# Sawyerbatch/simglucose

Measured on AMD Instinct MI355X. Metric: env-steps/sec at batch=1M patients (1-min dt); fp64 glucose trace max-abs-err, higher is better.
Workload: dtype f64

## Files before the change

### simglucose_amd/csrc/t1d_kernels.hpp

```cpp
#pragma once
#include "../../include/t1d.h"
#include "t1d_device.hpp"

#ifndef T1D_WAVES
#define T1D_WAVES 2
#endif
#ifndef T1D_ROW_RECOMPUTE
#define T1D_ROW_RECOMPUTE 1
#endif
constexpr int kFlagReverse = 0x10000;
#ifndef T1D_AB_FLAGS
#define T1D_AB_FLAGS 0
#endif

#include <climits>
#include <cstdint>
#include <type_traits>

namespace t1d {

template <typename T> struct KArgs {
    int64_t n, env_offset;
    uint64_t seed;
    T* x; T* planned; T* last_qsto; T* last_food; int32_t* t; uint32_t* meta; uint32_t* episode; int32_t* next_meal;
// ... 91 lines not shown
template <typename T>
__device__ __forceinline__ void stage_prop(const KArgs<T>& a, T* lds)
{
    const int tot = a.prop_rows * a.np_pad;
    for (int j = threadIdx.x; j < tot; j += blockDim.x) lds[j] = a.prop[j];
    __syncthreads();
}

template <typename T>
__device__ __forceinline__ void load_env(const KArgs<T>& a, unsigned i, uint32_t meta, Env<T>& e)
{
#pragma unroll
    for (int k = 0; k < 13; ++k) e.x[k] = at(row(a.x, a.n, k), i);
    e.planned = at(a.planned, i); e.lq = at(a.last_qsto, i); e.lf = at(a.last_food, i);
    e.last_cgm = at(a.last_cgm, i); e.prev_risk = at(a.prev_risk, i);
#pragma unroll
    for (int k = 0; k < 4; ++k) e.cur[k] = at(row(a.pts, a.n, 22 + k), i);
    e.t = at(a.t, i);
    e.next_meal = a.next_meal ? at(a.next_meal, i) : 0;
    e.next_meal_loaded = e.next_meal;
    e.eating = (meta & T1D_META_EATING) != 0;
    e.cursor = (int)T1D_META_CURSOR(meta);
}

template <typename T>
__device__ __forceinline__ void store_env(const KArgs<T>& a, unsigned i, uint32_t pid, const Env<T>& e)
{
#pragma unroll
    for (int k = 0; k < 13; ++k) at(row(a.x, a.n, k), i) = e.x[k];
    at(a.planned, i) = e.planned; at(a.last_qsto, i) = e.lq; at(a.last_food, i) = e.lf;
    at(a.last_cgm, i) = e.last_cgm; at(a.prev_risk, i) = e.prev_risk;
    if (a.dbar) at(a.dbar, i) = dbar_of(e.lq, e.lf);
    at(a.t, i) = e.t;
    if (a.next_meal && e.next_meal != e.next_meal_loaded) at(a.next_meal, i) = e.next_meal;
    at(a.meta, i) = pid | (e.eating ? T1D_META_EATING : 0u) | (e.planned > T(0) ? T1D_META_PLANNED : 0u) | ((uint32_t)e.cursor << 16);
}

constexpr int kPtsRows = 26;
constexpr int kPackedRows = 18 + kPtsRows + 1;
constexpr int kRowDbar = 18 + kPtsRows;

#ifndef T1D_REFILL_INLINE
#define T1D_REFILL_INLINE 1
#endif
#if T1D_REFILL_INLINE
#define T1D_REFILL_ATTR __forceinline__
#else
#define T1D_REFILL_ATTR __noinline__
#endif

template <typename T>
__device__ T1D_REFILL_ATTR void noise_refill(T* __restrict__ pts, const T* __restrict__ normals, const T* __restrict__ minv,
                                             const uint32_t* __restrict__ episode, int* status, int64_t n, unsigned i,
                                             int64_t env_offset, uint64_t seed, int n_normals, int b, SensorC<T> sen, T* ar_e)
{
    const T p0 = at(rowv(pts, n, b > 0 ? 10 : 0), i);
    at(pts, i) = p0;
    T M[11];
#pragma unroll
    for (int k = 0; k < 11; ++k) M[k] = minv[k * 11] * p0;
    T e = *ar_e;
    const uint32_t ep = (!normals && episode) ? at(episode, i) : 0u;
#pragma unroll 1
    for (int q = 0; q < 5; ++q) {
        T z0, z1;
        if (normals) {
            const int d = 1 + 10 * b + 2 * q;
            if (d + 1 < n_normals) { z0 = at(rowv(normals, n, d), i); z1 = at(rowv(normals, n, d + 1), i); }
            else { z0 = z1 = T(0); atomicOr(status, T1D_ST_NORMALS_EXHAUSTED); }
        } else {
            const double2 r = philox_pair(seed, (uint64_t)(env_offset + i), ep, 3u + 5u * (uint32_t)b + (uint32_t)q);
            z0 = (T)r.x; z1 = (T)r.y;
        }
        e = sen.pacf * (e + z0);
        const T ya = johnson_su<true>(sen, e);
        e = sen.pacf * (e + z1);
        const T yb = johnson_su<true>(sen, e);
        at(rowv(pts, n, 2 * q + 1), i) = ya;
        at(rowv(pts, n, 2 * q + 2), i) = yb;
        const T* mc = minv + (2 * q + 1);
#pragma unroll
        for (int k = 0; k < 11; ++k) M[k] += mc[k * 11] * ya + mc[k * 11 + 1] * yb;
    }
    *ar_e = e;
#pragma unroll
    for (int k = 0; k < 11; ++k) at(rowv(pts, n, 11 + k), i) = M[k];
}

__device__ __forceinline__ void divmod_uniform(int x, int d, int& q, int& r)
{
    switch (d) {
        case 1: q = x; r = 0; return;
        case 3: q = x / 3; break;
        case 5: q = x / 5; break;
        case 30: q = x / 30; break;
        case 50: q = x / 50; break;
        case 150: q = x / 150; break;
        default: q = x / d; break;
    }
    r = x - q * d;
}

template <bool REFILL, typename T>
__device__ __forceinline__ T noise_sample(const KArgs<T>& a, unsigned i, int s, T (&cur)[4], bool* entered = nullptr)
{
    const int64_t n = a.n;
    const int st = a.sen.st;
    int j, b;
    divmod_uniform(s, a.S, b, j);
    const int tau = (j + 1) * st;
    const int m = tau / 15 < 9 ? tau / 15 : 9;
    const int mprev = (tau - st) / 15 < 9 ? (tau - st) / 15 : 9;
    if (REFILL && j == 0) {
        T e = at(a.ar_e, i);
        noise_refill<T>(a.pts, a.normals, a.minv, a.episode, a.status, n, i, a.env_offset, a.seed, a.n_normals, b, a.sen, &e);
        at(a.ar_e, i) = e;
    }
    if (j == 0 || m != mprev) {
        cur[0] = at(rowv(a.pts, n, m), i);      cur[1] = at(rowv(a.pts, n, m + 1), i);
        cur[2] = at(rowv(a.pts, n, 11 + m), i); cur[3] = at(rowv(a.pts, n, 12 + m), i);
        if (entered) *entered = true;
        else {
#pragma unroll
            for (int k = 0; k < 4; ++k) at(row(a.pts, n, 22 + k), i) = cur[k];
        }
    }
    const T B = T(tau - 15 * m) * T(1.0 / 15.0), A = fma(-T(tau - 15 * m), T(1.0 / 15.0), T(1));
    const T ca = fma(A * A, A, -A), cb = fma(B * B, B, -B);
    return fma(A, cur[0], fma(B, cur[1], T(37.5) * fma(ca, cur[2], cb * cur[3])));
}

template <bool REFILL, typename T>
__device__ __forceinline__ T measure_noise(const KArgs<T>& a, unsigned i, Env<T>& e, bool& due, bool* entered = nullptr)
{
    const int t1 = e.t + 1;
    int q, r;
    divmod_uniform(t1, a.sen.st, q, r);
    due = r == 0;
    return due ? noise_sample<REFILL>(a, i, 1 + q, e.cur, entered) : T(0);
}
template <typename T>
__device__ __forceinline__ T measure_apply(const KArgs<T>& a, Env<T>& e, T gsub, T noise, bool due)
{
    if (due) {
        T cgm = gsub + noise;
        cgm = cgm > a.sen.vmin ? cgm : a.sen.vmin;
        cgm = cgm < a.sen.vmax ? cgm : a.sen.vmax;
        e.last_cgm = cgm;
    }
    return e.last_cgm;
}

template <typename T, bool HAS_NEXT = false, typename E = Env<T>>
__device__ __forceinline__ T meal_lookup(const KArgs<T>& a, unsigned i, E& e)
{
    T meal = T(0);
    if (HAS_NEXT || a.next_meal) {
        if (e.next_meal <= e.t) {
            while (e.cursor < a.n_meals) {
                const int mt = at(rowv(a.meal_time, a.n, e.cursor), i);
                if (mt > e.t) { e.next_meal = mt; break; }
                if (mt == e.t) meal = at(rowv(a.meal_amt, a.n, e.cursor), i);
                ++e.cursor;
            }
            if (e.cursor >= a.n_meals) e.next_meal = INT_MAX;
            asm volatile("" : "+v"(meal));
        }
    } else if (e.cursor < a.n_meals) {
        int mt = at(rowv(a.meal_time, a.n, e.cursor), i);
        while (mt < e.t && ++e.cursor < a.n_meals) mt = at(rowv(a.meal_time, a.n, e.cursor), i);
        if (e.cursor < a.n_meals && mt == e.t) {
            meal = at(rowv(a.meal_amt, a.n, e.cursor), i);
            ++e.cursor;
        }
    }
    return meal;
}

template <int MATH, typename T, typename P, bool REFILL = true, typename PR = NoProp, bool TIERED = false>
__device__ __forceinline__ StepOut<T> step_body(const KArgs<T>& a, P& p, unsigned i, Env<T>& e,
                                                T basal, T bolus, bool has_bolus, PR pr = PR())
{
    T q_basal, q_bolus;
    if ((a.flags & T1D_BATCH_NO_PUMP) || ab_flag(a, 0x200)) {
        q_basal = basal; q_bolus = has_bolus ? bolus : T(0);
    } else {
        q_basal = pump_quantise(basal, a.pump.inc_basal, a.pump.min_basal, a.pump.max_basal);
        q_bolus = a.pump.min_bolus > T(0) ? a.pump.min_bolus : T(0);
        if (has_bolus) q_bolus = pump_quantise(bolus, a.pump.inc_bolus, a.pump.min_bolus, a.pump.max_bolus);
    }
    const T insulin = q_basal + q_bolus;
    const T div = T(a.minutes), inv_div = T(1) / div;
    StepOut<T> o{T(0), T(0), T(0), T(0)};
    for (int m = 0; m < a.minutes; ++m) {
        const T meal = a.cho ? at(row(a.cho, a.n, m), i) : meal_lookup(a, i, e);
        bool due;
        const T noise = ab_flag(a, 0x400) ? (due = false, T(0)) : measure_noise<REFILL>(a, i, e, due);
        MinuteIn<T> u = eat_minute<MATH, T>(p, e.x, meal, insulin, e.planned, e.lq, e.lf, e.eating);
        if constexpr (PR::kSplit) p.pin_split(); else p.pin();
        if (!ab_flag(a, 0x800)) {
            if constexpr (PR::kSplit && TIERED) split_minute_tiered(p, pr, u, e.x, a.n_sub);
            else if constexpr (PR::kSplit) split_level<1>(p, pr, u, e.x, a.n_sub);
            else rk4_minute<MATH>(p, u, e.x, a.n_sub);
        }
        e.t += 1;
        const T gsub = MATH == 0 ? e.x[12] / p(DP_VG) : e.x[12] * p(DP_IVG);
        const T cgm = measure_apply(a, e, gsub, noise, due);
        if (MATH == 0) { o.meal += meal / div; o.ins += insulin / div; o.bg += gsub / div; o.cgm += cgm / div; }
        else { o.meal += meal * inv_div; o.ins += insulin * inv_div; o.bg += gsub * inv_div; o.cgm += cgm * inv_div; }
    }
    if (MATH != 0 && a.minutes == 1) { o.ins = insulin; }
    return o;
}

template <int MATH, typename T>
__device__ __forceinline__ void write_outputs(const KArgs<T>& a, unsigned i, Env<T>& e, const StepOut<T>& o, T rp)
{
    T l, h, r, rc = T(0);
    if (!ab_flag(a, 0x100)) risk_index1<MATH>(o.cgm, l, h, rc);
    at(a.reward, i) = rp - rc;
    e.prev_risk = rc;
    at(a.cgm, i) = o.cgm; at(a.bg, i) = o.bg;
    at(a.done, i) = (o.bg < T(70) || o.bg > T(350)) ? 1 : 0;
    if (a.lbgi || a.hbgi || a.risk) {
        risk_index1<MATH>(o.bg, l, h, r);
        if (a.lbgi) at(a.lbgi, i) = l;
        if (a.hbgi) at(a.hbgi, i) = h;
        if (a.risk) at(a.risk, i) = r;
    }
    if (a.meal) at(a.meal, i) = o.meal;
    if (a.insulin) at(a.insulin, i) = o.ins;
    if (!(fabs((double)e.x[12]) <= 1.0e300)) atomicOr(a.status, T1D_ST_NONFINITE);
}

template <int VARIANT> struct VariantMath { static constexpr int value = VARIANT == 0 ? 0 : 1; };
template <int VARIANT> struct VariantInfo {
    static_assert(VARIANT == 0 || VARIANT == 3 || VARIANT == 4 || VARIANT == 6 || VARIANT == 7, "unknown kernel variant");
    static constexpr bool split = VARIANT == 4 || VARIANT == 6 || VARIANT == 7;
    static constexpr bool tiered = VARIANT == 6 || VARIANT == 7;
    static constexpr bool lds_pars = VARIANT == 0 || VARIANT == 7;
};
extern __shared__ __align__(16) unsigned char t1d_dyn_lds[];

template <int VARIANT, typename T, bool REFILL = true>
__global__ __launch_bounds__(kBlock, T1D_WAVES) void step_kernel(const KArgs<T> a)
{
    constexpr int MATH = VariantMath<VARIANT>::value;
    using VI = VariantInfo<VARIANT>;
    constexpr int kParRows = VI::split ? DP_COUNT : DP_RK4_COUNT;
    __shared__ T lds[VI::lds_pars ? kParRows * kMaxPatients : 1];
    if (VI::lds_pars) stage_pars(a, lds, kParRows);
    if (VI::split) stage_prop(a, (T*)t1d_dyn_lds);
    const unsigned i = blockIdx.x * kBlock + threadIdx.x;
    __builtin_assume(i < (1u << 28));
    if ((int64_t)i >= a.n) return;
    const uint32_t meta = at(a.meta, i);
    const uint32_t pid = T1D_META_PID(meta);
    Env<T> e;
    load_env(a, i, meta, e);
    const T basal = at(a.basal, i);
    const T bolus = a.bolus ? at(a.bolus, i) : T(0);
    const T rp = e.prev_risk;
    StepOut<T> o;
    if constexpr (VARIANT == 4 || VARIANT == 6) {
        ParsReg<T> p;
        p.load(a.dpar, (int)pid);
        o = step_body<MATH, T, ParsReg<T>, REFILL, PropLds<T>, VARIANT == 6>(a, p, i, e, basal, bolus, a.bolus != nullptr, PropLds<T>{(const T*)t1d_dyn_lds, a.np_pad, (int)pid});
    } else if constexpr (VARIANT == 7) {
        ParsLds<T> p{lds, (int)pid};
        o = step_body<MATH, T, ParsLds<T>, REFILL, PropLds<T>, true>(a, p, i, e, basal, bolus, a.bolus != nullptr, PropLds<T>{(const T*)t1d_dyn_lds, a.np_pad, (int)pid});
    } else if constexpr (VARIANT == 3) {
        ParsReg<T> p;
        p.load(a.dpar, (int)pid);
        o = step_body<MATH, T, ParsReg<T>, REFILL>(a, p, i, e, basal, bolus, a.bolus != nullptr);
    } else {
        ParsLds<T> p{lds, (int)pid};
        o = step_body<MATH, T, ParsLds<T>, REFILL>(a, p, i, e, basal, bolus, a.bolus != nullptr);
    }
    write_outputs<MATH>(a, i, e, o, rp);
    store_env(a, i, pid, e);
}

#ifndef T1D_S1_WAVES
#define T1D_S1_WAVES 3
#endif
#ifndef T1D_S1_TRACE
#define T1D_S1_TRACE 0
#endif
#ifndef T1D_S1_PHASE_PRIO
#define T1D_S1_PHASE_PRIO 3
#endif
#if T1D_S1_TRACE
#define S1_MARK(m) do { __builtin_amdgcn_s_waitcnt(0x0070); if (tr && (threadIdx.x & 63) == 0 && tk < 6) tr[tk * 8 + (m)] = (long long)wall_clock64(); } while (0)
#else
#define S1_MARK(m) do { } while (0)
#endif
template <typename T> constexpr int s1_threads();
#ifndef T1D_S1D_WAVES
#define T1D_S1D_WAVES 4
#endif
#ifndef T1D_S1D_WAVES_F32
#define T1D_S1D_WAVES_F32 4
#endif
template <typename T> constexpr int s1d_threads() { return 256 * (sizeof(T) == 4 ? T1D_S1D_WAVES_F32 : T1D_S1D_WAVES); }
template <typename T> constexpr int s1_threads() { return 256 * (sizeof(T) == 4 ? T1D_S1D_WAVES_F32 : T1D_S1_WAVES); }
template <typename T> struct S1In { uint32_t meta; int t, next_meal; T basal, bolus, planned, lq, lf, x[13]; };

template <typename T>
__device__ __forceinline__ S1In<T> s1_load(const KArgs<T>& a, unsigned i)
{
    const BRows<T> X(a.x, a.n, kPackedRows);
    const BRows<int32_t> I(a.t, a.n, 3);
    S1In<T> in;
    in.meta = (uint32_t)(int32_t)at(I(1), i);
    in.t = at(I(0), i);
    in.next_meal = at(I(2), i);
    in.basal = at(a.basal, i);
    in.bolus = a.bolus ? (T)at(a.bolus, i) : T(0);
    const T dbar = at(X(kRowDbar), i);
#pragma unroll
    for (int k = 0; k < 13; ++k) in.x[k] = at(X(k), i);
    if ((in.meta & (T1D_META_EATING | T1D_META_PLANNED)) || (T1D_AB_FLAGS && (a.flags & 0x1000))) {
        in.planned = at(X(13), i); in.lq = at(X(14), i); in.lf = at(X(15), i);
    } else {
        in.planned = T(0); in.lq = dbar; in.lf = T(0);
    }
    return in;
}

constexpr int kS1DPark = 128;
template <typename T>
__device__ __forceinline__ void s1_park(const S1In<T>& in, T* pt, int* pi, int slot)
{
#pragma unroll
    for (int k = 0; k < 13; ++k) pt[k * kS1DPark + slot] = in.x[k];
    pt[13 * kS1DPark + slot] = in.planned; pt[14 * kS1DPark + slot] = in.lq; pt[15 * kS1DPark + slot] = in.lf;
    pt[16 * kS1DPark + slot] = in.basal; pt[17 * kS1DPark + slot] = in.bolus;
    pi[slot] = (int)in.meta; pi[kS1DPark + slot] = in.t; pi[2 * kS1DPark + slot] = in.next_meal;
}
template <typename T>
__device__ __forceinline__ S1In<T> s1_unpark(const T* pt, const int* pi, int slot)
{
    S1In<T> in;
#pragma unroll
    for (int k = 0; k < 13; ++k) in.x[k] = pt[k * kS1DPark + slot];
    in.planned = pt[13 * kS1DPark + slot]; in.lq = pt[14 * kS1DPark + slot]; in.lf = pt[15 * kS1DPark + slot];
    in.basal = pt[16 * kS1DPark + slot]; in.bolus = pt[17 * kS1DPark + slot];
    in.meta = (uint32_t)pi[slot]; in.t = pi[kS1DPark + slot]; in.next_meal = pi[2 * kS1DPark + slot];
    return in;
}

template <typename T, int MODE> constexpr bool kS1DLean = sizeof(T) == 8 && (MODE == 2 || MODE == 3);
constexpr int kLcVmin = 6, kLcVmax = 7, kLcLimits = 8, kLcHc1 = kLcLimits, kLcHc2 = kLcHc1 + 5, kLcSize = kLcHc2 + 5;
constexpr int kLcHc(int level) { return level == 1 ? kLcHc1 : kLcHc2; }
template <typename T>
__device__ __forceinline__ void pump_lconst(const T* lconst, T basal, T bolus, bool has_bolus, T& q_basal, T& q_bolus)
{
    int z = 0;
    asm volatile("" : "+v"(z));
    const T* lc = lconst + z;
    q_basal = pump_quantise(basal, lc[0], lc[1], lc[2]);
    q_bolus = lc[4] > T(0) ? lc[4] : T(0);
    if (has_bolus) q_bolus = pump_quantise(bolus, lc[3], lc[4], lc[5]);
}
template <bool REG, typename T, int STRIDE, bool EXTRA, int MODE, typename ONLEVEL>
__device__ __forceinline__ void s1_chunk(const KArgs<T>& a, T* ldp, T* lpr, T* lconst, unsigned i, const S1In<T>& in,
                                         ONLEVEL&& on_level, long long* tr, int tk)
{
    constexpr int LEVEL = MODE == 3 ? 2 : 1;
    (void)tr; (void)tk;
    S1_MARK(0);
    const BRows<T> X(a.x, a.n, kPackedRows);
    const BRows<int32_t> I(a.t, a.n, 3);
    const uint32_t meta = in.meta;
    Env<T> e;
    e.t = in.t;
    e.next_meal = in.next_meal;
    const T basal = in.basal;
    const T bolus = in.bolus;
    e.planned = in.planned; e.lq = in.lq; e.lf = in.lf;
#pragma unroll
    for (int k = 0; k < 13; ++k) e.x[k] = in.x[k];
    const uint32_t pid = T1D_META_PID(meta);
    const T planned0 = e.planned, lq0 = e.lq, lf0 = e.lf;
    e.next_meal_loaded = e.next_meal;
    e.eating = (meta & T1D_META_EATING) != 0;
    e.cursor = (int)T1D_META_CURSOR(meta);
    S1_MARK(1);
    T q_basal, q_bolus;
    if (a.flags & T1D_BATCH_NO_PUMP) {
        q_basal = basal; q_bolus = a.bolus ? bolus : T(0);
    } else {
        pump_lconst(lconst, basal, bolus, a.bolus != nullptr, q_basal, q_bolus);
    }
    const T insulin = q_basal + q_bolus;
    T meal;
    if (a.cho) {
        meal = at(a.cho, i);
        asm volatile("" : "+v"(meal));
    } else {
        meal = meal_lookup<T, true>(a, i, e);
    }
    ParsLdsS<T, STRIDE> pl{ldp, (int)pid};
    MinuteIn<T> u = eat_minute<1, T>(pl, e.x, meal, insulin, e.planned, e.lq, e.lf, e.eating);
    T f1 = T(0);
    if (MODE == 2) {
        const TierPre<T> tp = tier_pre(pl, u, e.x);
        f1 = tp.f1;
        on_level(tp.level2);
        if (tp.level2) return;
    }
    {
        const bool live0 = (meta & (T1D_META_EATING | T1D_META_PLANNED)) != 0 || (T1D_AB_FLAGS && (a.flags & 0x1000));
        const bool changed = live0 ? (e.planned != planned0 || e.lq != lq0 || e.lf != lf0) : (e.eating || e.planned > T(0));
        if (changed) {
            at(X(13), i) = e.planned; at(X(14), i) = e.lq; at(X(15), i) = e.lf;
            at(X(kRowDbar), i) = dbar_of(e.lq, e.lf);
        }
    }
    at(I(0), i) = e.t + 1;
    if (e.next_meal != e.next_meal_loaded) at(I(2), i) = e.next_meal;
    {
        const uint32_t meta1 = pid | (e.eating ? T1D_META_EATING : 0u) | (e.planned > T(0) ? T1D_META_PLANNED : 0u) | ((uint32_t)e.cursor << 16);
        if (meta1 != meta) at(I(1), i) = (int32_t)meta1;
    }
    if (EXTRA) {
        if (a.meal) at(a.meal, i) = meal;
        if (a.insulin) at(a.insulin, i) = insulin;
    }
    S1_MARK(2);
#if T1D_S1_PHASE_PRIO
    if (MODE != 3) __builtin_amdgcn_s_setprio(0);
#endif
    if (!ab_flag(a, 0x800)) {
        PropLdsS<T, STRIDE> pr{lpr, (int)pid};
        if (MODE == 1) {
            split_minute_tiered(pl, pr, u, e.x, a.n_sub);
        } else if constexpr (kS1DLean<T, MODE>) {
            ParsLdsH<T, STRIDE> ph{ldp, (int)pid};
            split_level<LEVEL, T, ParsLdsH<T, STRIDE>, decltype(pr), MODE == 2, true>(ph, pr, u, e.x, a.n_sub, f1, false, lconst + kLcHc(LEVEL));
        } else if (REG) {
            ParsReg<T> p;
#pragma unroll
            for (int k = 0; k < (int)(sizeof(kSplitPars) / sizeof(int)); ++k) p.v[kSplitPars[k]] = pl(kSplitPars[k]);
#pragma unroll
            for (int k = 0; k < 4; ++k) p.v[kSplitW(LEVEL) + k] = pl(kSplitW(LEVEL) + k);
            p.pin_split();
            split_level<LEVEL, T, ParsReg<T>, decltype(pr), MODE == 2>(p, pr, u, e.x, a.n_sub, f1);
        } else {
            split_level<LEVEL, T, ParsLdsS<T, STRIDE>, decltype(pr), MODE == 2>(pl, pr, u, e.x, a.n_sub, f1);
        }
    }
    S1_MARK(3);
#if T1D_S1_PHASE_PRIO
    __builtin_amdgcn_s_setprio(T1D_S1_PHASE_PRIO);
#endif
#pragma unroll
    for (int k = 0; k < 13; ++k) at(X(k), i) = e.x[k];
#pragma unroll
    for (int k = 0; k < 4; ++k) e.cur[k] = at(X(40 + k), i);
    T last_cgm = a.sen.st == 1 ? T(0) : (T)at(X(16), i);
    const T rp = at(X(17), i);
    S1_MARK(4);
    bool due, entered = false;
    const T noise = measure_noise<false>(a, i, e, due, &entered);
    if (entered) {
#pragma unroll
        for (int k = 0; k < 4; ++k) at(X(40 + k), i) = e.cur[k];
    }
    const T gsub = e.x[12] * pl(DP_IVG);
    bool in_range = false;
    if (due) {
        T c = gsub + noise;
        int z = 0;
        asm volatile("" : "+v"(z));
        const T vmin = lconst[kLcVmin + z], vmax = lconst[kLcVmax + z];
        in_range = vmin > T(1) && vmax < T(__builtin_huge_val());
        c = c > vmin ? c : vmin;
        c = c < vmax ? c : vmax;
        last_cgm = c;
        if (a.sen.st != 1) at(X(16), i) = c;
    }
    const T cgm_out = last_cgm, bg_out = gsub;
    at(a.cgm, i) = cgm_out; at(a.bg, i) = bg_out;
    if (!(fabs((double)e.x[12]) <= 1.0e300)) atomicOr(a.status, T1D_ST_NONFINITE);
    T l, h, r, rc = T(0);
    if (!ab_flag(a, 0x100)) {
        if (__builtin_amdgcn_ballot_w64(!in_range) == 0ull) risk_index1<1, T, true>(cgm_out, l, h, rc);
        else risk_index1<1>(cgm_out, l, h, rc);
    }
    at(a.reward, i) = rp - rc;
    at(X(17), i) = rc;
    at(a.done, i) = (bg_out < T(70) || bg_out > T(350)) ? 1 : 0;
    if (EXTRA && (a.lbgi || a.hbgi || a.risk)) {
        risk_index1<1>(bg_out, l, h, r);
        if (a.lbgi) at(a.lbgi, i) = l;
        if (a.hbgi) at(a.hbgi, i) = h;
        if (a.risk) at(a.risk, i) = r;
    }
#if T1D_S1_TRACE
    if (tr && (threadIdx.x & 63) == 0 && tk < 6) tr[tk * 8 + 5] = (long long)wall_clock64();
#endif
    S1_MARK(6);
}

struct S1NoLevel { __device__ __forceinline__ void operator()(bool) const {} };

constexpr int kImgConst = kLcLimits;
template <typename T, int NT>
__device__ __forceinline__ void s1_stage_image(const KArgs<T>& a, T* ldp, T* lconst)
{
    typedef unsigned int u32x4 __attribute__((ext_vector_type(4)));
    const int words = (DP_COUNT + a.prop_rows) * 32;
    const int units = words * (int)sizeof(T) / 16;
    const u32x4* __restrict__ src = (const u32x4*)a.img;
    u32x4* dst = (u32x4*)ldp;
    for (int j0 = 0; j0 < units; j0 += 4 * NT) {
        u32x4 v[4];
#pragma unroll
        for (int k = 0; k < 4; ++k) {
            const int j = j0 + k * NT + (int)threadIdx.x;
            v[k] = j < units ? src[j] : u32x4{0u, 0u, 0u, 0u};
        }
#pragma unroll
        for (int k = 0; k < 4; ++k) {
            const int j = j0 + k * NT + (int)threadIdx.x;
            if (j < units) dst[j] = v[k];
        }
    }
    if (threadIdx.x < kImgConst) lconst[threadIdx.x] = a.img[words + threadIdx.x];
}

template <typename T, int STRIDE>
__device__ __forceinline__ void s1_stage_tables(const KArgs<T>& a, T* ldp, T* lpr, T* lconst)
{
    for (int j = threadIdx.x; j < DP_COUNT * STRIDE; j += (int)blockDim.x) {
        const int r = j / STRIDE, c = j % STRIDE;
        ldp[j] = c < a.np ? a.dpar[r * kMaxPatients + c] : T(0);
    }
    for (int j = threadIdx.x; j < a.prop_rows * STRIDE; j += (int)blockDim.x) {
        const int r = j / STRIDE, c = j % STRIDE;
        lpr[j] = c < a.np ? a.prop[r * a.np_pad + c] : T(0);
    }
    if (threadIdx.x == 0) {
        lconst[0] = a.pump.inc_basal; lconst[1] = a.pump.min_basal; lconst[2] = a.pump.max_basal;
        lconst[3] = a.pump.inc_bolus; lconst[4] = a.pump.min_bolus; lconst[5] = a.pump.max_bolus;
        lconst[kLcVmin] = a.sen.vmin; lconst[kLcVmax] = a.sen.vmax;
    }
}

template <typename T, int STRIDE, bool EXTRA, bool TIERED>
__global__ __launch_bounds__(s1_threads<T>(), 1) void step1_kernel(const KArgs<T> a, int nchunks)
{
    T* const ldp = (T*)t1d_dyn_lds;
    T* const lpr = ldp + DP_COUNT * STRIDE;
    __shared__ int queue;
    __shared__ T lconst[kLcLimits];
    if constexpr (STRIDE == 32) s1_stage_image<T, s1_threads<T>()>(a, ldp, lconst);
    else s1_stage_tables<T, STRIDE>(a, ldp, lpr, lconst);
    if (threadIdx.x == 0) queue = 0;
    __syncthreads();
    const int per_block = (nchunks + (int)gridDim.x - 1) / (int)gridDim.x;
    const int first = (int)blockIdx.x * per_block;
    const int count = nchunks - first < per_block ? nchunks - first : per_block;
    const unsigned lane = threadIdx.x & 63u;
#if T1D_S1_TRACE
    long long* tr = (a.trace && blockIdx.x < 32) ? a.trace + (blockIdx.x * (s1_threads<T>() / 64) + threadIdx.x / 64) * 64 : nullptr;
#else
    long long* tr = nullptr;
#endif
    int tk = -1;
    for (int it = 0;; ++it) {
        int c = 0;
        if (lane == 0) c = atomicAdd(&queue, 1);
        c = __builtin_amdgcn_readfirstlane(c);
        if (c >= count) break;
        const unsigned i = (unsigned)(first + c) * 64u + lane;
        __builtin_assume(i < (1u << 28));
        ++tk;
        if ((int64_t)i < a.n) s1_chunk<!TIERED, T, STRIDE, EXTRA, TIERED ? 1 : 0>(a, ldp, lpr, lconst, i, s1_load(a, i), S1NoLevel(), tr, tk);
    }
}

template <typename T, bool EXTRA>
__global__ __launch_bounds__(s1d_threads<T>(), 1) void step1d_kernel(const KArgs<T> a, int nchunks)
{
    constexpr int STRIDE = 32;
    T* const ldp = (T*)t1d_dyn_lds;
    T* const lpr = ldp + DP_COUNT * STRIDE;
    const int per_block = (nchunks + (int)gridDim.x - 1) / (int)gridDim.x;
    const unsigned lane = threadIdx.x & 63u;
    T* const park_t = lpr + a.prop_rows * STRIDE;
    int* const park_i = (int*)(park_t + 18 * kS1DPark);
    uint16_t* const list = (uint16_t*)(park_i + 3 * kS1DPark);
    __shared__ int queue, taken, listed, passed;
    __shared__ T lconst[kS1DLean<T, 2> ? kLcSize : kLcLimits];
    s1_stage_image<T, s1d_threads<T>()>(a, ldp, lconst);
    if (threadIdx.x == 0) { queue = 0; taken = 0; listed = 0; passed = 0; }
    if constexpr (kS1DLean<T, 2>) {
        if (threadIdx.x == 0) {
            T hc[5];
            split_step_sizes<T>(a.n_sub, hc);
            for (int k = 0; k < 5; ++k) lconst[kLcHc1 + k] = hc[k];
            split_step_sizes<T>(2 * a.n_sub, hc);
            for (int k = 0; k < 5; ++k) lconst[kLcHc2 + k] = hc[k];
        }
    }
    __syncthreads();
    const int first = (int)blockIdx.x * per_block;
    const int count = nchunks - first < per_block ? nchunks - first : per_block;
    const unsigned base = (unsigned)first * 64u;
    long long* tr = nullptr;
#if T1D_S1_TRACE
    long long* const ph = (a.trace && blockIdx.x < 32) ? a.trace + (blockIdx.x * (s1d_threads<T>() / 64) + threadIdx.x / 64) * 64 : nullptr;
#define S1D_PHASE(k) do { if (ph && lane == 0) ph[k] = (long long)wall_clock64(); } while (0)
#else
#define S1D_PHASE(k) do { } while (0)
#endif
    S1D_PHASE(0);
    auto draw = [&](int* counter) -> int {
        int g = 0;
        if (lane == 0) g = atomicAdd(counter, 1);
        return __builtin_amdgcn_readfirstlane(g);
    };
    auto on_level = [&](unsigned i, const S1In<T>& in) {
        return [&, i](bool level2) {
            if (level2) {
                const int slot = atomicAdd(&listed, 1);
                list[slot] = (uint16_t)(i - base);
                if (slot < kS1DPark) s1_park(in, park_t, park_i, slot);
            }
            __builtin_amdgcn_fence(__ATOMIC_RELEASE, "workgroup");
            if (lane == 0) atomicAdd(&passed, 1);
        };
    };
    int it = 0;
    for (;; ++it) {
        const int c = draw(&queue);
        if (c >= count) break;
        const unsigned i = (unsigned)(first + ((a.flags & kFlagReverse) ? count - 1 - c : c)) * 64u + lane;
        __builtin_assume(i < (1u << 28));
        if ((int64_t)i < a.n) {
#if T1D_S1_TRACE
            tr = ph ? ph + 16 : nullptr;
#endif
            const S1In<T> in = s1_load(a, i);
            s1_chunk<true, T, STRIDE, EXTRA, 2>(a, ldp, lpr, lconst, i, in, on_level(i, in), tr, it);
        }
    }
    tr = nullptr;
    S1D_PHASE(1);
    while (__hip_atomic_load(&passed, __ATOMIC_RELAXED, __HIP_MEMORY_SCOPE_WORKGROUP) < count) __builtin_amdgcn_s_sleep(4);
    __builtin_amdgcn_fence(__ATOMIC_ACQUIRE, "workgroup");
    __builtin_amdgcn_s_setprio(3);
    const int total = __hip_atomic_load(&listed, __ATOMIC_RELAXED, __HIP_MEMORY_SCOPE_WORKGROUP);
    S1D_PHASE(2);
#if T1D_S1_TRACE
    if (ph && lane == 0) { ph[6] = total; ph[7] = 0; ph[8] = it; }
#endif
    for (;;) {
        const int lo = draw(&taken) * 64;
        if (lo >= total) break;
        if (lo + (int)lane < total) {
            const unsigned i = base + (unsigned)list[lo + (int)lane];
            __builtin_assume(i < (1u << 28));
            const S1In<T> in = lo + 64 <= kS1DPark ? s1_unpark<T>(park_t, park_i, lo + (int)lane) : s1_load(a, i);
            s1_chunk<true, T, STRIDE, EXTRA, 3>(a, ldp, lpr, lconst, i, in, S1NoLevel(), nullptr, 0);
        }
    }
    __builtin_amdgcn_s_waitcnt(0x0070);
    S1D_PHASE(3);
    S1D_PHASE(4);
#undef S1D_PHASE
}

template <typename T> struct SnLane {
    T x[13];
    T planned, lq, lf, insulin, bg_sum, cgm_sum, meal_sum, last_cgm;
    int t, next_meal, cursor, m;
    unsigned i;
    uint32_t pid;
    int dirty;
    bool eating;
};
constexpr int kSnParkT = 21, kSnParkI = 5;
constexpr int kSnDirtyShift = 9;
constexpr int kSnSpinLimit = 1 << 20;

template <typename T>
__device__ __forceinline__ void sn_park(const SnLane<T>& L, T* pt, int* pi, int cap, int slot)
{
#pragma unroll
    for (int k = 0; k < 13; ++k) pt[k * cap + slot] = L.x[k];
    pt[13 * cap + slot] = L.planned; pt[14 * cap + slot] = L.lq; pt[15 * cap + slot] = L.lf; pt[16 * cap + slot] = L.insulin;
    pt[17 * cap + slot] = L.bg_sum; pt[18 * cap + slot] = L.cgm_sum; pt[19 * cap + slot] = L.meal_sum; pt[20 * cap + slot] = L.last_cgm;
    pi[slot] = (int)L.i; pi[cap + slot] = L.t; pi[2 * cap + slot] = L.next_meal;
    pi[3 * cap + slot] = (int)(L.pid | (L.eating ? T1D_META_EATING : 0u) | ((uint32_t)L.dirty << kSnDirtyShift) | ((uint32_t)L.cursor << 16));
    __builtin_amdgcn_fence(__ATOMIC_RELEASE, "workgroup");
    __hip_atomic_store(&pi[4 * cap + slot], L.m, __ATOMIC_RELAXED, __HIP_MEMORY_SCOPE_WORKGROUP);
}
__device__ __forceinline__ void sn_wait_records(int* pi, int cap, int lo, int n, unsigned lane, int* status)
{
    for (int spins = 0;; ++spins) {
        int m = 0;
        if ((int)lane < n) m = __hip_atomic_load(&pi[4 * cap + lo + (int)lane], __ATOMIC_RELAXED, __HIP_MEMORY_SCOPE_WORKGROUP);
        if (__builtin_amdgcn_ballot_w64(m < 0) == 0ull) break;
        if (spins > kSnSpinLimit) { if (lane == 0) atomicOr(status, T1D_ST_STALL); break; }
        __builtin_amdgcn_s_sleep(1);
    }
    __builtin_amdgcn_fence(__ATOMIC_ACQUIRE, "workgroup");
}
template <typename T>
__device__ __forceinline__ void sn_unpark(SnLane<T>& L, const T* pt, const int* pi, int cap, int slot)
{
#pragma unroll
    for (int k = 0; k < 13; ++k) L.x[k] = pt[k * cap + slot];
    L.planned = pt[13 * cap + slot]; L.lq = pt[14 * cap + slot]; L.lf = pt[15 * cap + slot]; L.insulin = pt[16 * cap + slot];
    L.bg_sum = pt[17 * cap + slot]; L.cgm_sum = pt[18 * cap + slot]; L.meal_sum = pt[19 * cap + slot]; L.last_cgm = pt[20 * cap + slot];
    L.i = (unsigned)pi[slot]; L.t = pi[cap + slot]; L.next_meal = pi[2 * cap + slot]; L.m = pi[4 * cap + slot];
    const uint32_t w = (uint32_t)pi[3 * cap + slot];
    L.pid = T1D_META_PID(w); L.eating = (w & T1D_META_EATING) != 0; L.dirty = (int)((w >> kSnDirtyShift) & 7u); L.cursor = (int)T1D_META_CURSOR(w);
    if (L.m < 0) L.m = 1 << 30;
}

#ifndef T1D_SN_WAVES
#define T1D_SN_WAVES 2
#endif
#ifndef T1D_SN_WAVES_F32
#define T1D_SN_WAVES_F32 4
#endif
template <typename T> constexpr int sn_threads() { return 256 * (sizeof(T) == 4 ? T1D_SN_WAVES_F32 : T1D_SN_WAVES); }
template <typename T, bool EXTRA, bool CTRL>
__global__ __launch_bounds__(sn_threads<T>(), 1) void stepn_kernel(const KArgs<T> a, const PidArgs<T> c, int nchunks, int park_cap, int mode)
{
    constexpr int STRIDE = 32;
    constexpr int NT = sn_threads<T>();
    T* const ldp = (T*)t1d_dyn_lds;
    T* const lpr = ldp + DP_COUNT * STRIDE;
    T* const park_t = lpr + a.prop_rows * STRIDE;
    int* const park_i = (int*)(park_t + kSnParkT * park_cap);
    const int per_block = (nchunks + (int)gridDim.x - 1) / (int)gridDim.x;
    unsigned long long* const redo = (unsigned long long*)(park_i + kSnParkI * park_cap + ((kSnParkI * park_cap) & 1));
    __shared__ int queue, taken, parked, passed, redo_any, redo_next;
    __shared__ T lconst[kLcSize + 2];
    s1_stage_tables<T, STRIDE>(a, ldp, lpr, lconst);
    const int first = (int)blockIdx.x * per_block;
    const int count = nchunks - first < per_block ? nchunks - first : per_block;
    const bool tiered = (mode & 1) != 0, all_redo = (mode & 2) != 0;
    const int group_min = mode >> 8;
    if (threadIdx.x == 0) {
        queue = 0; taken = 0; parked = 0; passed = all_redo ? count : 0; redo_any = 0; redo_next = 0;
        T hc[5];
        split_step_sizes<T>(a.n_sub, hc);
        for (int k = 0; k < 5; ++k) lconst[kLcHc1 + k] = hc[k];
        split_step_sizes<T>(2 * a.n_sub, hc);
        for (int k = 0; k < 5; ++k) lconst[kLcHc2 + k] = hc[k];
    }
    for (int j = threadIdx.x; j < park_cap; j += NT) park_i[4 * park_cap + j] = -1;
    for (int j = threadIdx.x; j < per_block; j += NT) {
        unsigned long long bits = 0ull;
        if (all_redo && j < count) {
            const int64_t left = a.n - (int64_t)(first + j) * 64;
            bits = left >= 64 ? ~0ull : (left > 0 ? (1ull << left) - 1ull : 0ull);
        }
        redo[j] = bits;
    }
    if (threadIdx.x == 0 && all_redo) redo_any = 1;
    __syncthreads();
    const unsigned lane = threadIdx.x & 63u;
    const BRows<T> X(a.x, a.n, kPackedRows);
    const BRows<int32_t> I(a.t, a.n, 3);
    const T inv_div = T(1) / T(a.minutes);
    const int st = a.sen.st;
    auto load_lane = [&](SnLane<T>& L, unsigned i) {
        const uint32_t meta = (uint32_t)(int32_t)at(I(1), i);
        L.t = at(I(0), i);
        L.next_meal = at(I(2), i);
        T basal = T(0), bolus = T(0);
        bool has_bolus = a.bolus != nullptr;
        T obs = T(0), k_integ = T(0), k_prev = T(0), bb_basal = T(0), bb_cr = T(1), bb_cf = T(1), prev_meal = T(0);
        if (CTRL) {
            obs = at(a.cgm, i);
            if (c.kind == 1) { bb_basal = at(c.bb_basal, i); bb_cr = at(c.bb_cr, i); bb_cf = at(c.bb_cf, i); prev_meal = at(c.bb_prev_meal, i); }
            else { k_integ = at(c.integ, i); k_prev = at(c.prev, i); }
        } else {
            basal = at(a.basal, i);
            if (has_bolus) bolus = at(a.bolus, i);
        }
        L.planned = at(X(13), i); L.lq = at(X(14), i); L.lf = at(X(15), i);
#pragma unroll
        for (int k = 0; k < 13; ++k) L.x[k] = at(X(k), i);
        L.last_cgm = st == 1 ? T(0) : (T)at(X(16), i);
        L.i = i; L.m = 0; L.dirty = 0;
        L.pid = T1D_META_PID(meta);
        L.eating = (meta & T1D_META_EATING) != 0;
        L.cursor = (int)T1D_META_CURSOR(meta);
        if (CTRL) {
            const T stT = T(st);
            has_bolus = true;
            if (c.kind == 1) {
                basal = bb_basal;
                if (prev_meal > T(0)) {
                    const T corr = obs > T(150) ? (obs - c.target) / bb_cf : T(0);
                    bolus = ((prev_meal * stT) / bb_cr + corr) / stT;
                }
            } else {
                basal = c.P * (obs - c.target) + c.I * k_integ + c.D * (obs - k_prev) / stT;
            }
        }
        T q_basal, q_bolus;
        if (a.flags & T1D_BATCH_NO_PUMP) {
            q_basal = basal; q_bolus = has_bolus ? bolus : T(0);
        } else {
            pump_lconst(lconst, basal, bolus, has_bolus, q_basal, q_bolus);
        }
        L.insulin = q_basal + q_bolus;
        L.bg_sum = T(0); L.cgm_sum = T(0); L.meal_sum = T(0);
    };
    auto minute_head = [&](SnLane<T>& L, T& meal, TierPre<T>& tp) -> MinuteIn<T> {
        if (a.cho) {
            meal = at(rowv(a.cho, a.n, L.m), L.i);
            asm volatile("" : "+v"(meal));
        } else {
            meal = meal_lookup<T, true>(a, L.i, L);
        }
        ParsLdsS<T, STRIDE> pl{ldp, (int)L.pid};
        MinuteIn<T> u = eat_minute<1, T>(pl, L.x, meal, L.insulin, L.planned, L.lq, L.lf, L.eating);
        if (tiered) tp = tier_pre(pl, u, L.x);
        else { tp.f1 = kgut_flux(pl, u, L.x[0], L.x[1]); tp.level2 = false; }
        return u;
    };
    auto gather_pars = [&](ParsReg<T>& p, uint32_t pid) {
        ParsLdsS<T, STRIDE> pl{ldp, (int)pid};
#pragma unroll
        for (int k = 0; k < (int)(sizeof(kSplitPars) / sizeof(int)); ++k) p.v[kSplitPars[k]] = pl(kSplitPars[k]);
#pragma unroll
        for (int k = 0; k < 4; ++k) p.v[kSplitW(1) + k] = pl(kSplitW(1) + k);
    };
    auto gather_pars2 = [&](ParsReg<T>& p, uint32_t pid) {
        gather_pars(p, pid);
        ParsLdsS<T, STRIDE> pl{ldp, (int)pid};
#pragma unroll
        for (int k = 0; k < 4; ++k) p.v[kSplitW(2) + k] = pl(kSplitW(2) + k);
    };
    auto integrate = [&](ParsReg<T>& p, SnLane<T>& L, const MinuteIn<T>& u, T f1) {
        PropLdsS<T, STRIDE> pr{lpr, (int)L.pid};
        p.pin_split();
        split_level<1, T, ParsReg<T>, decltype(pr), true, true>(p, pr, u, L.x, a.n_sub, f1, false, lconst + kLcHc1);
    };
    auto minute_tail = [&](SnLane<T>& L, T meal) {
        L.t += 1;
        ParsLdsS<T, STRIDE> pl{ldp, (int)L.pid};
        const T gsub = L.x[12] * pl(DP_IVG);
        int q, r;
        divmod_uniform(L.t, st, q, r);
        if (r == 0) {
            T cur[4];
#pragma unroll
            for (int k = 0; k < 4; ++k) cur[k] = at(X(40 + k), L.i);
            bool entered = false;
            const T noise = noise_sample<false>(a, L.i, 1 + q, cur, &entered);
            if (entered) {
#pragma unroll
                for (int k = 0; k < 4; ++k) at(X(40 + k), L.i) = cur[k];
            }
            int z = 0;
            asm volatile("" : "+v"(z));
            const T vmin = lconst[kLcVmin + z], vmax = lconst[kLcVmax + z];
            T cv = gsub + noise;
            cv = cv > vmin ? cv : vmin;
            cv = cv < vmax ? cv : vmax;
            L.last_cgm = cv;
        }
        L.meal_sum += meal * inv_div; L.bg_sum += gsub * inv_div; L.cgm_sum += L.last_cgm * inv_div;
    };
    auto epilogue = [&](SnLane<T>& L) {
        const unsigned i = L.i;
#pragma unroll
        for (int k = 0; k < 13; ++k) at(X(k), i) = L.x[k];
        if (L.dirty & 1) { at(X(13), i) = L.planned; at(X(14), i) = L.lq; at(X(15), i) = L.lf; at(X(kRowDbar), i) = dbar_of(L.lq, L.lf); }
        at(I(0), i) = L.t;
        if (L.dirty & 2) at(I(2), i) = L.next_meal;
        if (L.dirty & 5) at(I(1), i) = (int32_t)(L.pid | (L.eating ? T1D_META_EATING : 0u) | (L.planned > T(0) ? T1D_META_PLANNED : 0u) | ((uint32_t)L.cursor << 16));
        if (st != 1) at(X(16), i) = L.last_cgm;
        const T rp = at(X(17), i);
        const T cgm_out = L.cgm_sum, bg_out = L.bg_sum;
        if (CTRL && c.kind == 0) {
            const T obs = at(a.cgm, i);
            at(c.integ, i) = (T)at(c.integ, i) + (obs - c.target) * T(st);
            at(c.prev, i) = obs;
        }
        at(a.cgm, i) = cgm_out; at(a.bg, i) = bg_out;
        if (!(fabs((double)L.x[12]) <= 1.0e300)) atomicOr(a.status, T1D_ST_NONFINITE);
        T l, h, r = T(0), rc = T(0);
        risk_index1<1>(cgm_out, l, h, rc);
        at(a.reward, i) = rp - rc;
        at(X(17), i) = rc;
        at(a.done, i) = (bg_out < T(70) || bg_out > T(350)) ? 1 : 0;
        T ins_out = L.insulin;
        if (a.minutes != 1) {
            ins_out = T(0);
            for (int m = 0; m < a.minutes; ++m) ins_out += L.insulin * inv_div;
        }
        if (EXTRA) {
            const bool want_risk = a.lbgi || a.hbgi || a.risk || (CTRL && c.sum_risk);
            if (want_risk) risk_index1<1>(bg_out, l, h, r);
            if (a.lbgi) at(a.lbgi, i) = l;
            if (a.hbgi) at(a.hbgi, i) = h;
            if (a.risk) at(a.risk, i) = r;
            if (a.meal) at(a.meal, i) = L.meal_sum;
            if (a.insulin) at(a.insulin, i) = ins_out;
        }
        if (CTRL) {
            if (c.kind == 1) at(c.bb_prev_meal, i) = L.meal_sum;
            if (c.bg_trace) c.bg_trace[c.trace_row * a.n + i] = bg_out;
            if (c.cgm_trace) c.cgm_trace[c.trace_row * a.n + i] = cgm_out;
            if (c.cho_trace) c.cho_trace[c.trace_row * a.n + i] = L.meal_sum;
            if (c.ins_trace) c.ins_trace[c.trace_row * a.n + i] = ins_out;
            if (c.sum_risk) at(c.sum_risk, i) = (T)at(c.sum_risk, i) + r;
            if (c.min_bg) { const T v = at(c.min_bg, i); at(c.min_bg, i) = bg_out < v ? bg_out : v; }
            if (c.max_bg) { const T v = at(c.max_bg, i); at(c.max_bg, i) = bg_out > v ? bg_out : v; }
            if (c.n_low) at(c.n_low, i) = (int)at(c.n_low, i) + (bg_out < T(70) ? 1 : 0);
            if (c.n_high) at(c.n_high, i) = (int)at(c.n_high, i) + (bg_out > T(180) ? 1 : 0);
        }
    };
    for (;;) {
        int w_chunk = -1, w_lo = 0, w_n = 0, w_redo = -1;
        if (lane == 0) {
            bool full = false;
            if (!all_redo) {
                int pk = __hip_atomic_load(&parked, __ATOMIC_RELAXED, __HIP_MEMORY_SCOPE_WORKGROUP);
                pk = pk < park_cap ? pk : park_cap;
                int tk = __hip_atomic_load(&taken, __ATOMIC_RELAXED, __HIP_MEMORY_SCOPE_WORKGROUP);
                const int av = pk - tk < 64 ? pk - tk : 64;
                if (av >= group_min && __hip_atomic_compare_exchange_strong(&taken, &tk, tk + av, __ATOMIC_RELAXED, __ATOMIC_RELAXED, __HIP_MEMORY_SCOPE_WORKGROUP)) {
                    w_lo = tk; w_n = av; full = true;
                }
            }
            const int cc = (all_redo || full) ? count : atomicAdd(&queue, 1);
            if (cc < count) w_chunk = cc;
            else if (!full) {
                for (int spins = 0;; ++spins) {
                    const int ps = __hip_atomic_load(&passed, __ATOMIC_RELAXED, __HIP_MEMORY_SCOPE_WORKGROUP);
                    __builtin_amdgcn_fence(__ATOMIC_ACQUIRE, "workgroup");
                    int pk = __hip_atomic_load(&parked, __ATOMIC_RELAXED, __HIP_MEMORY_SCOPE_WORKGROUP);
                    pk = pk < park_cap ? pk : park_cap;
                    int tk = __hip_atomic_load(&taken, __ATOMIC_RELAXED, __HIP_MEMORY_SCOPE_WORKGROUP);
                    const int avail = pk - tk;
                    if (avail > 0) {
                        const int n = avail < 64 ? avail : 64;
                        if (__hip_atomic_compare_exchange_strong(&taken, &tk, tk + n, __ATOMIC_RELAXED, __ATOMIC_RELAXED, __HIP_MEMORY_SCOPE_WORKGROUP)) {
// ... 575 lines not shown
```

Before: 12.91 billion.

## Overlap table staging with first-chunk state loads in step1d kernel

Splits the LDS table-image staging into an issue phase (global loads into registers) and a land phase (LDS stores), so each wave's first chunk of patient state can be loaded while the table image is still in flight. Waves get their initial chunk statically (wave index), the shared queue counter is pre-advanced past those chunks, and the loop is restructured to consume a preloaded chunk before drawing the next. Out-of-range lanes load a clamped in-bounds index so loads can be issued unconditionally. This hides the kernel-prologue latency at the cost of more live registers during staging.

Measured after the change: 12.95 billion (median of 6 runs). About the same (+0.3%).

```diff
diff --git a/simglucose_amd/csrc/t1d_kernels.hpp b/simglucose_amd/csrc/t1d_kernels.hpp
--- a/simglucose_amd/csrc/t1d_kernels.hpp
+++ b/simglucose_amd/csrc/t1d_kernels.hpp
@@ -417,6 +417,9 @@
 #ifndef T1D_S1D_WAVES_F32
 #define T1D_S1D_WAVES_F32 4
 #endif
+#ifndef T1D_S1D_EARLY
+#define T1D_S1D_EARLY 4
+#endif
 template <typename T> constexpr int s1d_threads() { return 256 * (sizeof(T) == 4 ? T1D_S1D_WAVES_F32 : T1D_S1D_WAVES); }
 template <typename T> constexpr int s1_threads() { return 256 * (sizeof(T) == 4 ? T1D_S1D_WAVES_F32 : T1D_S1_WAVES); }
 template <typename T> struct S1In { uint32_t meta; int t, next_meal; T basal, bolus, planned, lq, lf, x[13]; };
@@ -442,6 +445,9 @@
     }
     return in;
 }
+
+template <typename T>
+__device__ __forceinline__ unsigned s1_load_env(const KArgs<T>& a, unsigned i) { return (int64_t)i < a.n ? i : i & ~63u; }
 
 constexpr int kS1DPark = 128;
 template <typename T>
@@ -644,6 +650,52 @@
         }
     }
     if (threadIdx.x < kImgConst) lconst[threadIdx.x] = a.img[words + threadIdx.x];
+}
+
+typedef unsigned int s1_u32x4 __attribute__((ext_vector_type(4)));
+template <typename T> struct S1Stage { s1_u32x4 v[4]; T lc; };
+
+template <typename T, int NT>
+__device__ __forceinline__ S1Stage<T> s1_stage_issue(const KArgs<T>& a)
+{
+    const int words = (DP_COUNT + a.prop_rows) * 32;
+    const int units = words * (int)sizeof(T) / 16;
+    const s1_u32x4* __restrict__ src = (const s1_u32x4*)a.img;
+    S1Stage<T> s;
+#pragma unroll
+    for (int k = 0; k < 4; ++k) {
+        const int j = k * NT + (int)threadIdx.x;
+        s.v[k] = j < units ? src[j] : s1_u32x4{0u, 0u, 0u, 0u};
+    }
+    s.lc = threadIdx.x < kImgConst ? a.img[words + threadIdx.x] : T(0);
+    return s;
+}
+
+template <typename T, int NT>
+__device__ __forceinline__ void s1_stage_land(const KArgs<T>& a, const S1Stage<T>& s, T* ldp, T* lconst)
+{
+    const int units = (DP_COUNT + a.prop_rows) * 32 * (int)sizeof(T) / 16;
+    const s1_u32x4* __restrict__ src = (const s1_u32x4*)a.img;
+    s1_u32x4* dst = (s1_u32x4*)ldp;
+#pragma unroll
+    for (int k = 0; k < 4; ++k) {
+        const int j = k * NT + (int)threadIdx.x;
+        if (j < units) dst[j] = s.v[k];
+    }
+    for (int j0 = 4 * NT; j0 < units; j0 += 4 * NT) {
+        s1_u32x4 v[4];
+#pragma unroll
+        for (int k = 0; k < 4; ++k) {
+            const int j = j0 + k * NT + (int)threadIdx.x;
+            v[k] = j < units ? src[j] : s1_u32x4{0u, 0u, 0u, 0u};
+        }
+#pragma unroll
+        for (int k = 0; k < 4; ++k) {
+            const int j = j0 + k * NT + (int)threadIdx.x;
+            if (j < units) dst[j] = v[k];
+        }
+    }
+    if (threadIdx.x < kImgConst) lconst[threadIdx.x] = s.lc;
 }
 
 template <typename T, int STRIDE>
@@ -701,17 +753,30 @@
 __global__ __launch_bounds__(s1d_threads<T>(), 1) void step1d_kernel(const KArgs<T> a, int nchunks)
 {
     constexpr int STRIDE = 32;
+    const unsigned lane = threadIdx.x & 63u;
+    long long* tr = nullptr;
+#if T1D_S1_TRACE
+    long long* const ph = (a.trace && blockIdx.x < 32) ? a.trace + (blockIdx.x * (s1d_threads<T>() / 64) + threadIdx.x / 64) * 64 : nullptr;
+#define S1D_PHASE(k) do { if (ph && lane == 0) ph[k] = (long long)wall_clock64(); } while (0)
+#else
+#define S1D_PHASE(k) do { } while (0)
+#endif
+    S1D_PHASE(5);
     T* const ldp = (T*)t1d_dyn_lds;
     T* const lpr = ldp + DP_COUNT * STRIDE;
     const int per_block = (nchunks + (int)gridDim.x - 1) / (int)gridDim.x;
-    const unsigned lane = threadIdx.x & 63u;
     T* const park_t = lpr + a.prop_rows * STRIDE;
     int* const park_i = (int*)(park_t + 18 * kS1DPark);
     uint16_t* const list = (uint16_t*)(park_i + 3 * kS1DPark);
     __shared__ int queue, taken, listed, passed;
     __shared__ T lconst[kS1DLean<T, 2> ? kLcSize : kLcLimits];
-    s1_stage_image<T, s1d_threads<T>()>(a, ldp, lconst);
-    if (threadIdx.x == 0) { queue = 0; taken = 0; listed = 0; passed = 0; }
+    const int first = (int)blockIdx.x * per_block;
+    const int count = nchunks - first < per_block ? nchunks - first : per_block;
+    const unsigned base = (unsigned)first * 64u;
+    auto env_of = [&](int c) -> unsigned { return (unsigned)(first + ((a.flags & kFlagReverse) ? count - 1 - c : c)) * 64u + lane; };
+    constexpr int kWaves = s1d_threads<T>() / 64;
+    const S1Stage<T> staged = s1_stage_issue<T, s1d_threads<T>()>(a);
+    if (threadIdx.x == 0) { queue = count < kWaves ? (count > 0 ? count : 0) : kWaves; taken = 0; listed = 0; passed = 0; }
     if constexpr (kS1DLean<T, 2>) {
         if (threadIdx.x == 0) {
             T hc[5];
@@ -721,17 +786,21 @@
             for (int k = 0; k < 5; ++k) lconst[kLcHc2 + k] = hc[k];
         }
     }
+    int c = __builtin_amdgcn_readfirstlane((int)(threadIdx.x >> 6));
+    unsigned i = 0;
+    S1In<T> in;
+    bool have = c < count && c < T1D_S1D_EARLY;
+    bool own = !have;
+    if (have) {
+        i = env_of(c);
+        __builtin_assume(i < (1u << 28));
+        in = s1_load(a, s1_load_env(a, i));
+        s1_stage_land<T, s1d_threads<T>()>(a, staged, ldp, lconst);
+        asm volatile("" ::: "memory");
+    } else {
+        s1_stage_land<T, s1d_threads<T>()>(a, staged, ldp, lconst);
+    }
     __syncthreads();
-    const int first = (int)blockIdx.x * per_block;
-    const int count = nchunks - first < per_block ? nchunks - first : per_block;
-    const unsigned base = (unsigned)first * 64u;
-    long long* tr = nullptr;
-#if T1D_S1_TRACE
-    long long* const ph = (a.trace && blockIdx.x < 32) ? a.trace + (blockIdx.x * (s1d_threads<T>() / 64) + threadIdx.x / 64) * 64 : nullptr;
-#define S1D_PHASE(k) do { if (ph && lane == 0) ph[k] = (long long)wall_clock64(); } while (0)
-#else
-#define S1D_PHASE(k) do { } while (0)
-#endif
     S1D_PHASE(0);
     auto draw = [&](int* counter) -> int {
         int g = 0;
@@ -750,18 +819,23 @@
         };
     };
     int it = 0;
-    for (;; ++it) {
-        const int c = draw(&queue);
+    for (;;) {
+        if (have) {
+            if ((int64_t)i < a.n) {
+#if T1D_S1_TRACE
+                tr = ph ? ph + 16 : nullptr;
+#endif
+                s1_chunk<true, T, STRIDE, EXTRA, 2>(a, ldp, lpr, lconst, i, in, on_level(i, in), tr, it);
+            }
+            ++it;
+        }
+        if (!own) c = draw(&queue);
+        own = false;
         if (c >= count) break;
-        const unsigned i = (unsigned)(first + ((a.flags & kFlagReverse) ? count - 1 - c : c)) * 64u + lane;
+        i = env_of(c);
         __builtin_assume(i < (1u << 28));
-        if ((int64_t)i < a.n) {
-#if T1D_S1_TRACE
-            tr = ph ? ph + 16 : nullptr;
-#endif
-            const S1In<T> in = s1_load(a, i);
-            s1_chunk<true, T, STRIDE, EXTRA, 2>(a, ldp, lpr, lconst, i, in, on_level(i, in), tr, it);
-        }
+        in = s1_load(a, s1_load_env(a, i));
+        have = true;
     }
     tr = nullptr;
     S1D_PHASE(1);
```
